# Tuee22/SpectralMC

Hardware: AMD Instinct MI355X
Metric: training-steps/sec (contracts*paths/s) + HBM GB/s, GBM 4096x65536 (higher is better)
Workload: dtype f32; 1 GPU; C2: 4096 contracts x 65536 paths (N=256 x M=256), T=16, 3-layer CVNN 6->32->32->256 fp32; contracts_per_gpu=4096, global_contracts=4096, network_size=256, batches_per_mc_run=256, assets=1, math=hw, parallelism=dp1

## Files before the change

### spectralmc_amd/csrc/gbm.hip

```cpp

#include <cmath>
#include <cstdlib>

#pragma clang fp contract(off)

#include "smc_internal.h"
#include "smc_sobol.h"
#include "smc_math.h"
#include "smc_rng.h"
#include "smc_device.h"

namespace smc {
namespace {

constexpr int kRowsWavesF64 = 4;
constexpr int kRowsWaves = 8;
constexpr int kThreads = 512;
constexpr int kWaves = kThreads / 64;
constexpr int kPathsPerLane = 4;
constexpr int kChunk = kThreads * kPathsPerLane;
constexpr double kLog2e = 1.4426950408889634;
constexpr size_t kMaxLds = 160 * 1024;

struct Contract {
  double X0, K, T, r, d, v;
};

struct EngineArgs {
  const double* contracts;
  int64_t B;
  int32_t T;
  int64_t P;
  int32_t N, M;
  uint64_t seed;
  const int64_t* ordinal_dev;
  int64_t ordinal0;
  int32_t scheme;
  int32_t normalize;
  int32_t store;
  int32_t simulate;
  int32_t all_rows;
  void* paths;
  double* rowsum;
  void* targets;
  int64_t pitch;
  int32_t slices;
  double* partials;
  uint32_t* arrivals;
  uint32_t* queues;
  const uint32_t* sobol;
  int32_t sobol_dim;
  const double* lower;
  const double* upper;
  double* contracts_out;
  float* cvnn_out;
  int64_t* cursor;
  int64_t sobol_index0;
  int64_t advance;
  uint32_t* done;
  int32_t res_slices;
  int32_t res_groups;
  uint32_t* res_cnt;
  double* res_xsum;
  double* res_xcol;
  uint32_t* res_queue;
  int32_t res_static_q = 3;
  uint32_t* status;
  uint32_t* launch_fail;
  uint32_t spin_limit;
  int32_t withhold;
};

constexpr int kSliceChunks = 4;



template <typename Real>
struct Vec4T;
template <>
struct Vec4T<float> {
  using type = float4;
};
template <>
struct Vec4T<double> {
  using type = double4;
};


__device__ __forceinline__ Contract load_contract(const double* c) {
  return Contract{c[0], c[1], c[2], c[3], c[4], c[5]};
}

__device__ __forceinline__ double wave_sum(double x) {
#pragma unroll
  for (int off = 32; off >= 1; off >>= 1) x += __shfl_xor(x, off, 64);
  return x;
}

template <typename Real, bool LOG_EULER, bool HW>
struct Stepper {
  Real a, b;

  static constexpr double zscale() {
    return sizeof(Real) == 4 && HW ? PathStream::kNormalScale<true> : 1.0;
  }

  __device__ Stepper(const Contract& c, int T) {
    const double dt = c.T / static_cast<double>(T);
    const double sq = sqrt(dt);
    if (LOG_EULER) {
      const double drift = c.r - c.d - 0.5 * c.v * c.v;
      const double scale = sizeof(Real) == 4 ? kLog2e : math::kExpUnit;
      a = static_cast<Real>(drift * dt * scale);
      b = static_cast<Real>(c.v * sq * scale * zscale());
    } else {
      a = static_cast<Real>((c.r - c.d) * dt);
      b = static_cast<Real>(c.v * sq * zscale());
    }
  }

  __device__ __forceinline__ Real operator()(Real x, Real z) const {
    if constexpr (LOG_EULER) {
      if constexpr (sizeof(Real) == 4 && HW) return x * __builtin_amdgcn_exp2f(fmaf(b, z, a));
      else if constexpr (sizeof(Real) == 4) return x * math::exp2_any(fmaf(b, z, a));
      else return math::mul_exp2s_f64(x, fma(b, z, a));
    }
    if constexpr (sizeof(Real) == 4) return fabsf(fmaf(x, fmaf(b, z, a), x));
    else return fabs(fma(x, fma(b, z, a), x));
  }
};

constexpr int kRowBlock = 16;

template <typename Real>
__device__ __forceinline__ void advance_packed(Real (&x)[4], const Real (&y)[4]) {
  typedef float f2 __attribute__((ext_vector_type(2)));
#pragma unroll
  for (int j = 0; j < 4; j += 2) {
    const f2 e = {__builtin_amdgcn_exp2f(y[j]), __builtin_amdgcn_exp2f(y[j + 1])};
    const f2 v = f2{x[j], x[j + 1]} * e;
    x[j] = v.x;
    x[j + 1] = v.y;
  }
}

template <typename Real, bool LOG_EULER, bool HW, bool ALLROWS, bool MASKED, bool FULLBLOCK, bool STRAIGHT = false,
          bool STRAIGHT_ALL = true>
__device__ __forceinline__ void lane_paths(const EngineArgs& a, const Stepper<Real, LOG_EULER, HW>& step, Real x0,
                                           uint64_t ordinal, int64_t chunk, int nvalid, int t0, int nrows,
                                           Real* contract_base, double (&acc)[ALLROWS ? kRowBlock : 1],
                                           Real* x_out = nullptr, int lid = -1) {
  using V4 = typename Vec4T<Real>::type;
  const int T = a.T;
  const int64_t P = a.P;
  const int64_t pitch = a.pitch ? a.pitch : P;
  const bool store_all = STRAIGHT ? STRAIGHT_ALL : a.store == SMC_STORE_ALL;
  const int lane_id = lid < 0 ? static_cast<int>(threadIdx.x) : lid;
  const int64_t p0 = chunk + kPathsPerLane * static_cast<int64_t>(lane_id);
  PathStream s(a.seed, ordinal, static_cast<uint64_t>(p0 / kPathsPerLane), T);
  constexpr bool kPacked = HW && LOG_EULER && sizeof(Real) == 4;
  constexpr bool kY64 = LOG_EULER && sizeof(Real) == 8;
  Real x[kPathsPerLane], zl[kPathsPerLane], zh[kPathsPerLane];
#pragma unroll
  for (int j = 0; j < kPathsPerLane; ++j) x[j] = x0;
  for (int t = 0; t < (STRAIGHT ? 0 : t0); t += 2) {
    if constexpr (kPacked) {
      s.hw_log_increments4(step.b, step.a, zl, zh);
      advance_packed(x, zl);
      advance_packed(x, zh);
    } else if constexpr (kY64) {
      s.f64_log_increments4(step.b, step.a, zl, zh);
#pragma unroll
      for (int j = 0; j < kPathsPerLane; ++j) x[j] = math::mul_exp2s_f64(math::mul_exp2s_f64(x[j], zl[j]), zh[j]);
    } else {
#pragma unroll
      for (int j = 0; j < kPathsPerLane; ++j) s.template normal_pair<HW>(zl[j], zh[j]);
#pragma unroll
      for (int j = 0; j < kPathsPerLane; ++j) x[j] = step(step(x[j], zl[j]), zh[j]);
    }
  }
  const uint32_t lane_off = static_cast<uint32_t>(kPathsPerLane * sizeof(Real)) * static_cast<uint32_t>(lane_id);
  Real* chunk_base = contract_base + chunk;
  const __amdgpu_buffer_rsrc_t contract_rsrc = row_rsrc(contract_base);
#pragma unroll
  for (int i = 0; i < kRowBlock; ++i) {
    if (FULLBLOCK || i < nrows) {
      const int t = STRAIGHT ? i : t0 + i;
      const bool tail = !FULLBLOCK && t + 1 == T;
// ... 144 lines not shown
    advance(zh);
    hook(x, t + 1);
    if constexpr (STORE_ALL) store();
    row += rstride;
  }
  if (T & 1) {
    if constexpr (kPacked) s.hw_log_tail4(step.b, step.a, zl);
    else if constexpr (kY64) s.f64_log_tail4(step.b, step.a, zl);
    else s.template normal_tail<HW>(zl);
    advance(zl);
    hook(x, T - 1);
    if constexpr (STORE_ALL) store();
  }
  if constexpr (!STORE_ALL && STORE) store();
  Real part = 0;
#pragma unroll
  for (int j = 0; j < kPathsPerLane; ++j) {
    part += x[j];
    x_out[j] = x[j];
  }
  acc += static_cast<double>(part);
}

template <typename Real, bool LOG_EULER, bool HW, bool ALLROWS>
__device__ void simulate_contract(const EngineArgs& a, const Contract& c, uint64_t ordinal, int64_t b,
                                  int64_t p_begin, int64_t p_end, double* lds_acc, double* lds_tot) {
  const int tid = threadIdx.x, lane = tid & 63, wave = tid >> 6;
  const int T = a.T;
  const int64_t P = a.P;
  const bool store_all = a.store == SMC_STORE_ALL;
  const int64_t pitch = a.pitch ? a.pitch : P;
  Real* base = static_cast<Real*>(a.paths) + (store_all ? b * T * pitch : b * pitch);
  const bool vec_ok = (P % kPathsPerLane) == 0;
  const int64_t full_end = vec_ok ? p_begin + ((p_end - p_begin) / kChunk) * kChunk : p_begin;
  const Stepper<Real, LOG_EULER, HW> step(c, T);
  const Real x0 = static_cast<Real>(c.X0);
  constexpr int kAcc = ALLROWS ? kRowBlock : 1;

  for (int t0 = 0; t0 < T; t0 += kRowBlock) {
    const int nrows = T - t0 < kRowBlock ? T - t0 : kRowBlock;
    double acc[kAcc];
#pragma unroll
    for (int i = 0; i < kAcc; ++i) acc[i] = 0.0;
    int64_t chunk = p_begin;
    if (nrows == kRowBlock) {
      if (T == kRowBlock && store_all) {
        for (; chunk < full_end; chunk += kChunk)
          lane_paths<Real, LOG_EULER, HW, ALLROWS, false, true, true>(a, step, x0, ordinal, chunk, kPathsPerLane, 0,
                                                                      kRowBlock, base, acc);
      }
      for (; chunk < full_end; chunk += kChunk)
        lane_paths<Real, LOG_EULER, HW, ALLROWS, false, true>(a, step, x0, ordinal, chunk, kPathsPerLane, t0, nrows,
                                                              base, acc);
    }
    for (; chunk < p_end; chunk += kChunk) {
      const int64_t p0 = chunk + kPathsPerLane * tid;
      const int nvalid = static_cast<int>(p0 >= p_end ? 0 : (p_end - p0 >= kPathsPerLane ? kPathsPerLane : p_end - p0));
      lane_paths<Real, LOG_EULER, HW, ALLROWS, true, false>(a, step, x0, ordinal, chunk, nvalid, t0, nrows, base,
                                                            acc);
    }
    if (ALLROWS || t0 + nrows == T) {
#pragma unroll
      for (int i = 0; i < kAcc; ++i) {
        if (i < nrows) {
          const double w = wave_sum(acc[i]);
          if (lane == 0) lds_acc[wave * kRowBlock + i] = w;
        }
      }
      __syncthreads();
      const int first = ALLROWS ? 0 : nrows - 1;
      if (tid >= first && tid < nrows) {
        double tot = 0.0;
        for (int w = 0; w < kWaves; ++w) tot += lds_acc[w * kRowBlock + (ALLROWS ? tid : 0)];
        lds_tot[t0 + tid] = tot;
      }
      __syncthreads();
    }
  }
}

template <typename Real>
struct PayoffPre {
  Real F, df, K;
  __device__ explicit PayoffPre(const Contract& c) {
    const Real Tm = static_cast<Real>(c.T);
    if constexpr (sizeof(Real) == 4) {
      F = static_cast<float>(c.X0) * math::exp_any(static_cast<float>(c.r - c.d) * Tm);
      df = math::exp_any(static_cast<float>(-c.r) * Tm);
    } else {
      F = c.X0 * exp((c.r - c.d) * Tm);
      df = exp(-c.r * Tm);
    }
    K = static_cast<Real>(c.K);
  }
};

template <typename Real>
struct Payoff {
  Real s, K, df;
  Payoff() = default;
  __device__ Payoff(const EngineArgs& a, const Contract& c, double terminal_sum)
      : Payoff(a, PayoffPre<Real>(c), terminal_sum) {}
  __device__ Payoff(const EngineArgs& a, const PayoffPre<Real>& pre, double terminal_sum) {
    df = pre.df;
    s = a.normalize ? pre.F / static_cast<Real>(terminal_sum / static_cast<double>(a.P)) : Real(1);
    K = pre.K;
    if (terminal_sum != terminal_sum) df = static_cast<Real>(__builtin_nan(""));
  }
  __device__ __forceinline__ Real operator()(Real x) const {
    const Real xs = x * s;
    const Real diff = K - xs;
    return df * (diff > Real(0) ? diff : Real(0));
  }
};

template <typename Real>
__device__ void dft_row(const double* avg, const double* cs, const double* sn, int N,
                        typename Complex2<Real>::type* out, int tid = threadIdx.x, int nthreads = kThreads) {
  using C2 = typename Complex2<Real>::type;
  const int kmax = N / 2;
  const bool fuse_nyq = (N % 2) == 0 && kmax > 0 && kmax % nthreads == 0;
  for (int k = tid; k < kmax || (!fuse_nyq && k == kmax); k += nthreads) {
    const bool nyq = fuse_nyq && k == 0;
    double re = 0.0, im = 0.0, rq = 0.0, iq = 0.0;
    int idx = 0, iqx = 0;
    for (int n = 0; n < N; ++n) {
      re = fma(avg[n], cs[idx], re);
      im = fma(-avg[n], sn[idx], im);
      idx += k;
      if (idx >= N) idx -= N;
      if (nyq) {
        rq = fma(avg[n], cs[iqx], rq);
        iq = fma(-avg[n], sn[iqx], iq);
        iqx += kmax;
        if (iqx >= N) iqx -= N;
      }
    }
    C2 v;
    v.x = static_cast<Real>(re);
    v.y = static_cast<Real>(im);
    out[k] = v;
    if (k != 0 && 2 * k != N) {
      v.y = static_cast<Real>(-im);
      out[N - k] = v;
    }
    if (nyq) {
      v.x = static_cast<Real>(rq);
      v.y = static_cast<Real>(iq);
      out[kmax] = v;
    }
  }
}

template <int kBatch>
__device__ __forceinline__ void quad_column_sums(const float* row, const Payoff<float>& pay, int N, int M,
                                                 int cols, int G, double* part, int tid, int nthreads) {
  typedef float v4f __attribute__((ext_vector_type(4)));
  const __amdgpu_buffer_rsrc_t rsrc =
      __builtin_amdgcn_make_buffer_rsrc(const_cast<float*>(row), static_cast<short>(0), 0x7fffffff, 0x00020000);
  const int items = cols * G;
  for (int item = tid; item < items; item += nthreads) {
    const int q = item % cols, g = item / cols;
    double sum[4] = {0.0, 0.0, 0.0, 0.0};
    for (int m0 = g; m0 < M; m0 += G * kBatch) {
      v4f v[kBatch];
#pragma unroll
// ... 251 lines not shown
#pragma unroll
    for (int j = 0; j < kPathsPerLane; ++j) {
      s.template normal_pair<HWN>(zl[j], zh[j]);
      if constexpr (HWN) {
        zl[j] *= kz;
        zh[j] *= kz;
      }
    }
    advance(zl);
    if constexpr (STORE_ALL) store();
    row += rstride;
    advance(zh);
    if constexpr (STORE_ALL) store();
    row += rstride;
  }
  if (T & 1) {
    s.template normal_tail<HWN>(zl);
    if constexpr (HWN) {
#pragma unroll
      for (int j = 0; j < kPathsPerLane; ++j) zl[j] *= kz;
    }
    advance(zl);
    if constexpr (STORE_ALL) store();
  }
  if constexpr (!STORE_ALL) store();
  float part = 0.0f;
#pragma unroll
  for (int j = 0; j < kPathsPerLane; ++j) part += j < nvalid ? static_cast<float>(x[j]) : 0.0f;
  acc += static_cast<double>(part);
}

constexpr int kRowsRefWaves = 6;
template <bool LOG_EULER, bool STORE_ALL, bool HWN>
__global__ __launch_bounds__(kThreads) __attribute__((amdgpu_waves_per_eu(kRowsRefWaves)))
void rows_ref_kernel(EngineArgs a) {
  extern __shared__ double lds[];
  math::f64_tables_load();
  const int64_t ord0 = (a.ordinal_dev ? *a.ordinal_dev : 0) + a.ordinal0;
  const int64_t pitch = a.pitch ? a.pitch : a.P;
  const int T = a.T;
  int parity = 0;
  for (int64_t b = blockIdx.x; b < a.B; b += gridDim.x, parity ^= 1) {
    const Contract c = load_contract(a.contracts + b * 6);
    const Stepper<double, LOG_EULER, false> step(c, T);
    float* base = static_cast<float*>(a.paths) + (STORE_ALL ? b * T * pitch : b * pitch);
    double acc = 0.0;
    for (int64_t chunk = 0; chunk < a.P; chunk += kChunk)
      lane_rows_ref<LOG_EULER, STORE_ALL, HWN>(a, step, c.X0, static_cast<uint64_t>(ord0 + b), chunk, base, T, pitch, acc);
    const double w = wave_sum(acc);
    double* ws = lds + parity * kWaves;
    if ((threadIdx.x & 63) == 0) ws[threadIdx.x >> 6] = w;
    lds_barrier();
    if (threadIdx.x == 0) {
      double tot = 0.0;
      for (int k = 0; k < kWaves; ++k) tot += ws[k];
      *pad_sum<float>(a, b) = tot;
    }
  }
}

__device__ __forceinline__ double group_sum(const double* part, int n, int G, int N) {
  double t = 0.0;
  for (int g0 = 0; g0 < G; g0 += 8) {
    double v[8];
#pragma unroll
    for (int u = 0; u < 8; ++u) v[u] = part[(g0 + u < G ? g0 + u : G - 1) * N + n];
#pragma unroll
    for (int u = 0; u < 8; ++u)
      if (g0 + u < G) t += v[u];
  }
  return t;
}

constexpr int kResThreads = 1024;
constexpr int kResWaves = kResThreads / 64;
constexpr int kResChunk = kResThreads * kPathsPerLane;
constexpr int kResMaxChunks = 16;
constexpr int kResLdsChunks = 8;
constexpr int kResRegChunks = kResMaxChunks - kResLdsChunks;
constexpr size_t kResTermBytes = static_cast<size_t>(kResLdsChunks) * kResThreads * 16;
constexpr int kResMaxSlices = 8;

constexpr int kResPreDraw = 32;
constexpr int kResMaxT = 1 << 16;

size_t resident_lds_bytes(int N) {
  return kResTermBytes +
         (static_cast<size_t>(kResWaves) + 3 * static_cast<size_t>(N) + 9 + 6 * kResPreDraw) * sizeof(double);
}

__device__ __forceinline__ void column_sums_tree(const double* part, double* red, double* avg, int N, int M) {
  const int tid = threadIdx.x, lane = tid & 63, wave = tid >> 6;
  const int R = kResThreads / N;
  const int n = tid % N, k = tid / N;
  double p = 0.0;
  if (tid < N * R) {
#pragma unroll
    for (int u = 0; u < 4; ++u) p += part[(k + u * R) * N + n];
  }
  for (int off = 32; off >= N; off >>= 1) p += __shfl_xor(p, off, 64);
  lds_barrier();
  if (N < 64) {
    if (lane < N) red[wave * N + n] = p;
  } else if (tid < N * R) {
    red[k * N + n] = p;
  }
  lds_barrier();
  const int terms = N < 64 ? kResWaves : R;
  for (int c = tid; c < N; c += kResThreads) {
    double t = 0.0;
    for (int w = 0; w < terms; ++w) t += red[w * N + c];
    avg[c] = t / static_cast<double>(M);
  }
}

template <bool LOG_EULER, bool HW, bool STORE_ALL, bool T16, bool ONTHEFLY = false>
__global__ __launch_bounds__(kResThreads) void resident_kernel(EngineArgs a) {
  static_assert(!(ONTHEFLY && T16), "the on-the-fly CF phase is instantiated for the rolled row loop only");
  typedef float v4f __attribute__((ext_vector_type(4)));
  extern __shared__ double lds[];
  const int tid = threadIdx.x, lane = tid & 63, wave = tid >> 6;
  const int N = a.N, M = a.M;
  const int64_t P = a.P;
  const int64_t pitch = a.pitch ? a.pitch : P;
  const int W = a.res_slices > 1 ? a.res_slices : 1;
  int grp = blockIdx.x, slc = 0;
  if (W > 1) {
    if (gridDim.x % (8 * W) == 0) {
      slc = static_cast<int>((blockIdx.x >> 3) % W);
      grp = static_cast<int>((blockIdx.x & 7) + 8 * (blockIdx.x / (8 * W)));
    } else {
      slc = static_cast<int>(blockIdx.x % W);
      grp = static_cast<int>(blockIdx.x / W);
    }
  }
  const int groups = static_cast<int>(gridDim.x) / W;
  const int nch = static_cast<int>(P / (static_cast<int64_t>(W) * kResChunk));
  const int cols = N / 4;
  const int G = kResChunk / N;
  const int q = tid % cols, g = tid / cols;
  v4f* term_lds = reinterpret_cast<v4f*>(lds);
  double* part = lds;
  double* wsum = lds + kResTermBytes / sizeof(double);
  double* avg = wsum + kResWaves;
  double* cs = avg + N;
  double* sn = cs + N;
  double* row = sn + N;
  double* pre = row + 9;
  for (int j = tid; j < N; j += kResThreads) math::twiddle(j, N, sn[j], cs[j]);
  const int64_t ord0 = (a.ordinal_dev ? *a.ordinal_dev : 0) + a.ordinal0;
  const int64_t sob0 = a.sobol ? a.cursor[0] + a.sobol_index0 : 0;
  uint32_t round = 0;
  const int64_t n_static0 = (a.B / groups) * a.res_static_q / 4 * groups;
  const bool dyn = a.res_queue != nullptr && (W == 1 || n_static0 > 0);
  const int64_t n_static = dyn ? n_static0 : a.B;
  auto grab = [&]() -> int64_t {
    if (tid == 0) reinterpret_cast<int64_t*>(row + 8)[0] = n_static + atomicAdd(a.res_queue, 1u);
    lds_barrier();
    return reinterpret_cast<const int64_t*>(row + 8)[0];
  };
  auto next = [&](int64_t b) -> int64_t {
    if (b + groups < n_static) return b + groups;
    if (!dyn) return a.B;
    if (W == 1) return grab();
    return reinterpret_cast<const int64_t*>(row + 8)[0];
  };
  int64_t n_pre = 0;
  if (a.sobol) {
    const int64_t mine = grp < n_static ? (n_static - 1 - grp) / groups + 1 : 0;
    n_pre = mine < kResPreDraw ? mine : kResPreDraw;
    for (int t = tid; t < n_pre * 6; t += kResThreads) {
      const int k = t / 6, d = t % 6;
      const int64_t bb = grp + static_cast<int64_t>(k) * groups;
      const double v = sobol_coord(a.sobol, a.sobol_dim, d, static_cast<uint64_t>(sob0 + bb), a.lower, a.upper);
      pre[t] = v;
      if (slc == 0) {
        a.contracts_out[bb * 6 + d] = v;
        if (a.cvnn_out) a.cvnn_out[bb * 6 + d] = static_cast<float>(v);
      }
    }
    lds_barrier();
  }
  for (int64_t b = grp < n_static ? grp : (dyn ? grab() : a.B); b < a.B; b = next(b), ++round) {
    Contract c;
    if (a.sobol && static_cast<int64_t>(round) < n_pre) {
      const double* r = pre + static_cast<int64_t>(round) * 6;
      c = Contract{r[0], r[1], r[2], r[3], r[4], r[5]};
    } else if (a.sobol) {
      if (tid < 6) {
        const double v = sobol_coord(a.sobol, a.sobol_dim, tid, static_cast<uint64_t>(sob0 + b), a.lower, a.upper);
        row[tid] = v;
        if (slc == 0) {
          a.contracts_out[b * 6 + tid] = v;
          if (a.cvnn_out) a.cvnn_out[b * 6 + tid] = static_cast<float>(v);
        }
      }
      lds_barrier();
      c = Contract{row[0], row[1], row[2], row[3], row[4], row[5]};
    } else {
      c = load_contract(a.contracts + b * 6);
    }
    const int T = T16 ? kRowBlock : a.T;
    const Stepper<float, LOG_EULER, HW> step(c, T);
    const float x0 = static_cast<float>(c.X0);
    float* base = static_cast<float*>(a.paths) + (STORE_ALL ? b * T * pitch : b * pitch);
    const int64_t p0 = static_cast<int64_t>(slc) * nch * kResChunk;
    float term[kResRegChunks][kPathsPerLane];
    double acc[1] = {0.0};
    double colsum[kPathsPerLane] = {0.0, 0.0, 0.0, 0.0};
    const PayoffPre<float> pre(c);
    const Payoff<float> pay_raw(a, pre, 1.0);
    for (int ch = 0; ch < nch; ++ch) {
      float xt[kPathsPerLane];
      if constexpr (T16)
        lane_paths<float, LOG_EULER, HW, false, false, true, true, STORE_ALL>(
            a, step, x0, static_cast<uint64_t>(ord0 + b), p0 + static_cast<int64_t>(ch) * kResChunk, kPathsPerLane,
            0, kRowBlock, base, acc, xt);
      else
        lane_rows<float, LOG_EULER, HW, STORE_ALL>(a, step, x0, static_cast<uint64_t>(ord0 + b),
                                            p0 + static_cast<int64_t>(ch) * kResChunk, base, T, pitch, acc[0], xt);
      if constexpr (ONTHEFLY) {
#pragma unroll
        for (int j = 0; j < kPathsPerLane; ++j) colsum[j] += static_cast<double>(pay_raw(xt[j]));
      } else if (ch < kResLdsChunks) {
        term_lds[ch * kResThreads + tid] = v4f{xt[0], xt[1], xt[2], xt[3]};
      } else {
#pragma unroll
        for (int i = 0; i + 1 < kResRegChunks; ++i)
#pragma unroll
          for (int j = 0; j < kPathsPerLane; ++j) term[i][j] = term[i + 1][j];
#pragma unroll
        for (int j = 0; j < kPathsPerLane; ++j) term[kResRegChunks - 1][j] = xt[j];
      }
    }
    const double w = wave_sum(acc[0]);
    if (lane == 0) wsum[wave] = w;
    lds_barrier();
    double tot = 0.0;
    {
      double wv[kResWaves];
#pragma unroll
      for (int k = 0; k < kResWaves; ++k) wv[k] = wsum[k];
#pragma unroll
      for (int k = 0; k < kResWaves; ++k) tot += wv[k];
    }
    const int64_t xslot = (static_cast<int64_t>(grp) * 2 + (round & 1)) * (W + 1);
    if (W > 1) {
      if (tid == 0) {
        put_sc1(a.res_xsum + xslot + slc, tot);
        if (dyn && slc == 0 && b + groups >= n_static)
          put_sc1(reinterpret_cast<int64_t*>(a.res_xsum + xslot + W), n_static + atomicAdd(a.res_queue, 1u));
        asm volatile("s_waitcnt vmcnt(0)" ::: "memory");
        uint32_t* cnt = a.res_cnt + static_cast<int64_t>(grp) * 64;
        if (!(a.withhold && grp == 0 && slc == W - 1 && round == 0))
          __hip_atomic_fetch_add(cnt, 1u, __ATOMIC_RELAXED, __HIP_MEMORY_SCOPE_AGENT);
        const uint32_t want = static_cast<uint32_t>(W) * (round + 1);
        uint32_t spins = 0;
        bool ok;
        while (!(ok = get_sc1(cnt) >= want) && get_sc1(a.launch_fail) == 0u && ++spins < a.spin_limit)
          __builtin_amdgcn_s_sleep(2);
        if (!ok) {
          __hip_atomic_fetch_or(a.status, SMC_SYNC_EXCHANGE_TIMEOUT, __ATOMIC_RELAXED, __HIP_MEMORY_SCOPE_AGENT);
          __hip_atomic_store(a.launch_fail, 1u, __ATOMIC_RELAXED, __HIP_MEMORY_SCOPE_AGENT);
        }
        const double t = ordered_sum_wt(a.res_xsum + xslot, 0, W, 1);
        row[6] = ok ? t : __builtin_nan("");
        if (dyn && b + groups >= n_static)
          reinterpret_cast<int64_t*>(row + 8)[0] =
              ok ? get_sc1(reinterpret_cast<const int64_t*>(a.res_xsum + xslot + W)) : a.B;
      }
      lds_barrier();
      tot = row[6];
    }
    const Payoff<float> pay(a, pre, tot);
    if constexpr (!ONTHEFLY) {
#pragma unroll
      for (int j = 0; j < kPathsPerLane; ++j) colsum[j] = 0.0;
      v4f v[kResLdsChunks];
#pragma unroll
      for (int ch = 0; ch < kResLdsChunks; ++ch) v[ch] = term_lds[ch * kResThreads + tid];
#pragma unroll
      for (int ch = 0; ch < kResLdsChunks; ++ch) {
        if (ch < nch) {
#pragma unroll
          for (int j = 0; j < kPathsPerLane; ++j) colsum[j] += static_cast<double>(pay(v[ch][j]));
        }
      }
    }
#pragma unroll
    for (int i = 0; i < kResRegChunks && !ONTHEFLY; ++i) {
      if (i >= kResRegChunks - (nch - kResLdsChunks)) {
#pragma unroll
        for (int j = 0; j < kPathsPerLane; ++j) colsum[j] += static_cast<double>(pay(term[i][j]));
      }
    }
    lds_barrier();
#pragma unroll
    for (int j = 0; j < kPathsPerLane; ++j) part[g * N + 4 * q + j] = colsum[j];
    lds_barrier();
    if (W == 1) {
      column_sums_tree(part, part, avg, N, M);
    } else {
      for (int n = tid; n < N; n += kResThreads) {
        const double t = group_sum(part, n, G, N);
        avg[n] = t;
      }
      lds_barrier();
      double* xcol = a.res_xcol + xslot * N;
      if (wave == 0) {
        for (int n = lane; n < N; n += 64) put_sc1(xcol + static_cast<int64_t>(slc) * N + n, avg[n]);
        asm volatile("s_waitcnt vmcnt(0)" ::: "memory");
        if (lane == 0) {
          const uint32_t before = __hip_atomic_fetch_add(a.res_cnt + static_cast<int64_t>(grp) * 64 + 32, 1u,
                                                         __ATOMIC_RELAXED, __HIP_MEMORY_SCOPE_AGENT);
          reinterpret_cast<int*>(row + 7)[0] = before == static_cast<uint32_t>(W) * (round + 1) - 1;
        }
      }
      lds_barrier();
      if (!reinterpret_cast<const int*>(row + 7)[0]) continue;
      for (int n = tid; n < N; n += kResThreads) avg[n] = ordered_sum_wt(xcol, n, W, N) / static_cast<double>(M);
    }
    lds_barrier();
    fft_row<float, kResThreads, true>(avg, cs, sn, N, part, part + N, static_cast<float2*>(a.targets) + b * N);
    lds_barrier();
  }
  if (a.done && tid == 0) {
    __threadfence();
    if (atomicAdd(a.done, 1u) == gridDim.x - 1) {
      a.cursor[0] += a.advance;
      a.cursor[1] += a.advance;
      if (a.res_queue) *a.res_queue = 0u;
      if (W > 1) {
        for (int k = 0; k < groups; ++k) {
          a.res_cnt[static_cast<int64_t>(k) * 64] = 0u;
          a.res_cnt[static_cast<int64_t>(k) * 64 + 32] = 0u;
        }
        *a.launch_fail = 0u;
      }
      *a.done = 0u;
    }
  }
}

constexpr int kPackMinP = 256, kPackMaxP = 2048;

size_t packed_lds_bytes(int64_t P, int N) {
  const int64_t K = kResChunk / P;
  const int64_t part = K * P > 2 * K * N ? K * P : 2 * K * N;
  return static_cast<size_t>(part + K * N + 2 * N + kResWaves + 7 * K) * sizeof(double);
}

template <bool LOG_EULER, bool HW, bool STORE_ALL, bool T16>
__global__ __launch_bounds__(kResThreads) void packed_kernel(EngineArgs a) {
  extern __shared__ double lds[];
  const int tid = threadIdx.x, lane = tid & 63, wave = tid >> 6;
  const int N = a.N, M = a.M;
  const int64_t P = a.P;
  const int64_t pitch = a.pitch ? a.pitch : P;
  const int lpc = static_cast<int>(P / kPathsPerLane);
  const int K = kResThreads / lpc;
  const int wpc = lpc / 64;
  const int k = tid / lpc, l = tid - k * lpc;
  const int cols = N / 4;
  const int q = l % cols, g = l / cols;
  const int64_t partn = K * P > 2 * K * N ? K * P : 2 * static_cast<int64_t>(K) * N;
  double* part = lds;
  double* avg = part + partn;
  double* cs = avg + K * N;
  double* sn = cs + N;
  double* wsum = sn + N;
  double* rows = wsum + kResWaves;
  for (int j = tid; j < N; j += kResThreads) math::twiddle(j, N, sn[j], cs[j]);
  const int64_t ord0 = (a.ordinal_dev ? *a.ordinal_dev : 0) + a.ordinal0;
  const int64_t sob0 = a.sobol ? a.cursor[0] + a.sobol_index0 : 0;
  const int64_t ngroups = (a.B + K - 1) / K;
  for (int64_t grp = blockIdx.x; grp < ngroups; grp += gridDim.x) {
    const int64_t b0 = grp * K;
    const int kv = a.B - b0 < K ? static_cast<int>(a.B - b0) : K;
    if (tid < 6 * kv) {
      const int kk = tid / 6, d = tid - 6 * kk;
      double v;
      if (a.sobol) {
        v = sobol_coord(a.sobol, a.sobol_dim, d, static_cast<uint64_t>(sob0 + b0 + kk), a.lower, a.upper);
        a.contracts_out[(b0 + kk) * 6 + d] = v;
        if (a.cvnn_out) a.cvnn_out[(b0 + kk) * 6 + d] = static_cast<float>(v);
      } else {
        v = a.contracts[(b0 + kk) * 6 + d];
      }
      rows[kk * 7 + d] = v;
    }
    lds_barrier();
    const bool active = k < kv;
    const double* r = rows + (active ? k : 0) * 7;
    const Contract c{r[0], r[1], r[2], r[3], r[4], r[5]};
    const int T = T16 ? kRowBlock : a.T;
    float xt[kPathsPerLane] = {0.0f, 0.0f, 0.0f, 0.0f};
    double acc[1] = {0.0};
    if (active) {
      const Stepper<float, LOG_EULER, HW> step(c, T);
      const float x0 = static_cast<float>(c.X0);
      const int64_t b = b0 + k;
      float* base = static_cast<float*>(a.paths) + (STORE_ALL ? b * T * pitch : b * pitch);
      if constexpr (T16)
        lane_paths<float, LOG_EULER, HW, false, false, true, true, STORE_ALL>(
            a, step, x0, static_cast<uint64_t>(ord0 + b), 0, kPathsPerLane, 0, kRowBlock, base, acc, xt, l);
      else
        lane_rows<float, LOG_EULER, HW, STORE_ALL>(a, step, x0, static_cast<uint64_t>(ord0 + b), 0, base, T, pitch,
                                                   acc[0], xt, l);
    }
    const double w = wave_sum(acc[0]);
    if (lane == 0) wsum[wave] = w;
    lds_barrier();
    if (tid < K) {
      double tot = 0.0;
      for (int v = 0; v < wpc; ++v) tot += wsum[tid * wpc + v];
// ... 868 lines not shown

size_t workspace_bytes(int64_t B, int32_t T, int64_t P, bool all_rows) {
  const int64_t W = slices_for(P, true);
  if (W <= 1) return 0;
  return static_cast<size_t>(B) * W * (all_rows ? T : 1) * sizeof(double) + static_cast<size_t>(B + 16) * sizeof(uint32_t);
}

constexpr int kPathsWgsPerCu = 4;

template <bool LOG_EULER, bool HW, bool STRAIGHT, bool STORE_ALL>
int32_t launch_split_k(const EngineArgs& a, hipStream_t stream) {
  const size_t lds1 = lds_bytes(a.T, a.N, false), lds2 = lds_bytes(a.T, a.N, true);
  auto k1 = paths_kernel<LOG_EULER, HW, STRAIGHT, STORE_ALL>;
  auto k2 = cf_kernel<float>;
  if ((lds1 > 64 * 1024 && hipFuncSetAttribute(reinterpret_cast<const void*>(k1),
                                                hipFuncAttributeMaxDynamicSharedMemorySize,
                                                static_cast<int>(lds1)) != hipSuccess) ||
      (lds2 > 64 * 1024 && hipFuncSetAttribute(reinterpret_cast<const void*>(k2),
                                                hipFuncAttributeMaxDynamicSharedMemorySize,
                                                static_cast<int>(lds2)) != hipSuccess)) {
    (void)hipGetLastError();
    return fail(SMC_ERR_HIP, "paths_kernel / cf_kernel: cannot raise the dynamic LDS limit");
  }
  unsigned grid1 = static_cast<unsigned>(a.B);
  if (STRAIGHT) {
    int dev = 0, cus = 0;
    if (hipGetDevice(&dev) != hipSuccess ||
        hipDeviceGetAttribute(&cus, hipDeviceAttributeMultiprocessorCount, dev) != hipSuccess || cus <= 0) {
      (void)hipGetLastError();
      return fail(SMC_ERR_HIP, "paths_kernel: device query failed");
    }
    const int64_t slots = static_cast<int64_t>(kPathsWgsPerCu) * cus;
    if (slots < a.B) grid1 = static_cast<unsigned>(slots);
  }
  launch(k1, dim3(grid1), dim3(kThreads), lds1, stream, a);
  if (int32_t st = check_launch("paths_kernel")) return st;
  launch(k2, dim3(static_cast<unsigned>(a.B)), dim3(kThreads), lds2, stream, a);
  return check_launch("cf_kernel");
}

template <typename Real, bool LOG_EULER, bool HW, bool STORE_ALL>
int32_t launch_rows_k(const EngineArgs& a, hipStream_t stream) {
  const size_t lds1 = 2 * kWaves * sizeof(double), lds2 = lds_bytes(a.T, a.N, true);
  auto k1 = rows_kernel<Real, LOG_EULER, HW, STORE_ALL>;
  auto k2 = cf_kernel<Real>;
  if (lds2 > kMaxLds) return fail(SMC_ERR_INVALID_SHAPE, "engine: network_size exceeds the LDS budget");
  if (lds2 > 64 * 1024 && hipFuncSetAttribute(reinterpret_cast<const void*>(k2),
                                               hipFuncAttributeMaxDynamicSharedMemorySize,
                                               static_cast<int>(lds2)) != hipSuccess) {
    (void)hipGetLastError();
    return fail(SMC_ERR_HIP, "cf_kernel: cannot raise the dynamic LDS limit");
  }
  unsigned grid1 = 0;
  if (int32_t st = resident_grid(reinterpret_cast<const void*>(k1), kThreads, lds1, a.B, &grid1)) return st;
  launch(k1, dim3(grid1), dim3(kThreads), lds1, stream, a);
  if (int32_t st = check_launch("rows_kernel")) return st;
  launch(k2, dim3(static_cast<unsigned>(a.B)), dim3(kThreads), lds2, stream, a);
  return check_launch("cf_kernel");
}

template <bool LOG_EULER, bool STORE_ALL, bool HWN>
int32_t launch_rows_ref_k(const EngineArgs& a, hipStream_t stream) {
  const size_t lds1 = 2 * kWaves * sizeof(double), lds2 = lds_bytes(a.T, a.N, true);
  auto k1 = rows_ref_kernel<LOG_EULER, STORE_ALL, HWN>;
  auto k2 = cf_kernel<float>;
  if (lds2 > kMaxLds) return fail(SMC_ERR_INVALID_SHAPE, "engine: network_size exceeds the LDS budget");
  if (lds2 > 64 * 1024 && hipFuncSetAttribute(reinterpret_cast<const void*>(k2),
                                               hipFuncAttributeMaxDynamicSharedMemorySize,
                                               static_cast<int>(lds2)) != hipSuccess) {
    (void)hipGetLastError();
    return fail(SMC_ERR_HIP, "cf_kernel: cannot raise the dynamic LDS limit");
  }
  unsigned grid1 = 0;
  if (int32_t st = resident_grid(reinterpret_cast<const void*>(k1), kThreads, lds1, a.B, &grid1)) return st;
  launch(k1, dim3(grid1), dim3(kThreads), lds1, stream, a);
  if (int32_t st = check_launch("rows_ref_kernel")) return st;
  launch(k2, dim3(static_cast<unsigned>(a.B)), dim3(kThreads), lds2, stream, a);
  return check_launch("cf_kernel");
}

template <bool LOG_EULER, bool HW, bool STORE_ALL>
int32_t launch_resident_k(const EngineArgs& a, hipStream_t stream) {
  const int W = a.res_slices > 1 ? a.res_slices : 1;
  auto kernel = a.T == kRowBlock                 ? resident_kernel<LOG_EULER, HW, STORE_ALL, true>
                : (!a.normalize && W == 1) ? resident_kernel<LOG_EULER, HW, STORE_ALL, false, true>
                                           : resident_kernel<LOG_EULER, HW, STORE_ALL, false>;
  const size_t lds = resident_lds_bytes(a.N);
  if (lds > 64 * 1024 && hipFuncSetAttribute(reinterpret_cast<const void*>(kernel),
                                             hipFuncAttributeMaxDynamicSharedMemorySize,
                                             static_cast<int>(lds)) != hipSuccess) {
    (void)hipGetLastError();
    return fail(SMC_ERR_HIP, "resident_kernel: cannot raise the dynamic LDS limit");
  }
  unsigned grid = 0;
  if (int32_t st = resident_grid(reinterpret_cast<const void*>(kernel), kResThreads, lds, a.B * W, &grid, stream))
    return st;
  if (W > 1) {
    unsigned groups = grid / W;
    if (groups > static_cast<unsigned>(a.res_groups)) groups = static_cast<unsigned>(a.res_groups);
    if (groups >= 8) groups -= groups % 8;
    if (groups == 0) return fail(SMC_ERR_INVALID_SHAPE, "resident_kernel: fewer resident slots than slices");
    grid = groups * W;
  }
  launch(kernel, dim3(grid), dim3(kResThreads), lds, stream, a);
  return check_launch("resident_kernel");
}

template <bool LOG_EULER, bool HW, bool STORE_ALL>
int32_t launch_wave_k(const EngineArgs& a, hipStream_t stream) {
  auto kernel = a.T == 1 ? wave_kernel<LOG_EULER, HW, STORE_ALL, 1> : wave_kernel<LOG_EULER, HW, STORE_ALL, 2>;
  const size_t lds = wave_lds_bytes(a.N);
  if (lds > 64 * 1024 && hipFuncSetAttribute(reinterpret_cast<const void*>(kernel),
                                             hipFuncAttributeMaxDynamicSharedMemorySize,
                                             static_cast<int>(lds)) != hipSuccess) {
    (void)hipGetLastError();
    return fail(SMC_ERR_HIP, "wave_kernel: cannot raise the dynamic LDS limit");
  }
  unsigned grid = 0;
  const int64_t wpg = kWaveThreads / 64;
  if (int32_t st = resident_grid(reinterpret_cast<const void*>(kernel), kWaveThreads, lds, (a.B + wpg - 1) / wpg, &grid,
                                 stream))
    return st;
  launch(kernel, dim3(grid), dim3(kWaveThreads), lds, stream, a);
  return check_launch("wave_kernel");
}

template <bool LOG_EULER, bool HW, bool STORE_ALL>
int32_t launch_packed_k(const EngineArgs& a, hipStream_t stream) {
  auto kernel = a.T == kRowBlock ? packed_kernel<LOG_EULER, HW, STORE_ALL, true>
                                 : packed_kernel<LOG_EULER, HW, STORE_ALL, false>;
  const size_t lds = packed_lds_bytes(a.P, a.N);
  if (lds > kMaxLds) return fail(SMC_ERR_INVALID_SHAPE, "packed_kernel: network_size exceeds the LDS budget");
  if (lds > 64 * 1024 && hipFuncSetAttribute(reinterpret_cast<const void*>(kernel),
                                             hipFuncAttributeMaxDynamicSharedMemorySize,
                                             static_cast<int>(lds)) != hipSuccess) {
    (void)hipGetLastError();
    return fail(SMC_ERR_HIP, "packed_kernel: cannot raise the dynamic LDS limit");
  }
  const int64_t K = kResChunk / a.P;
  unsigned grid = 0;
  if (int32_t st = resident_grid(reinterpret_cast<const void*>(kernel), kResThreads, lds, (a.B + K - 1) / K, &grid,
                                 stream))
    return st;
  launch(kernel, dim3(grid), dim3(kResThreads), lds, stream, a);
  return check_launch("packed_kernel");
}


template <typename Real>
int32_t launch_engine(EngineArgs a, hipStream_t stream) {
  if (a.B == 0) return SMC_OK;
  if ((a.scheme & SMC_MATH_REF) != 0) {
    if (sizeof(Real) != 4) return fail(SMC_ERR_INVALID_ARGUMENT, "engine: SMC_MATH_REF is an f32 mode");
    if (!ref_ok(a))
      return fail(SMC_ERR_INVALID_SHAPE, "engine: SMC_MATH_REF needs targets, whole contracts per workgroup and "
                                         "a padded pitch (smc_path_pitch)");
    const bool log_euler = (a.scheme & 0xff) == SMC_SCHEME_LOG_EULER;
    const bool sa = a.store == SMC_STORE_ALL;
    if ((a.scheme & SMC_MATH_HW) != 0) {
      if (log_euler)
        return sa ? launch_rows_ref_k<true, true, true>(a, stream) : launch_rows_ref_k<true, false, true>(a, stream);
      return sa ? launch_rows_ref_k<false, true, true>(a, stream) : launch_rows_ref_k<false, false, true>(a, stream);
    }
    if (log_euler)
      return sa ? launch_rows_ref_k<true, true, false>(a, stream) : launch_rows_ref_k<true, false, false>(a, stream);
    return sa ? launch_rows_ref_k<false, true, false>(a, stream) : launch_rows_ref_k<false, false, false>(a, stream);
  }
  if constexpr (sizeof(Real) == 4) {
    if (wave_ok(a, true)) {
// ... 712 lines not shown
```

Baseline: 99.97 billion contracts*paths/s.

## Overlap next-contract prep and single-wave FFT in resident kernel, split sliced variant

Adds a SLICED template parameter so the unsliced resident kernel compiles without the cross-slice branches. In the unsliced path, one dedicated wave computes the next contract's stepper and payoff constants (Sobol draw, queue ticket) into LDS while wave 0 performs the column mean and FFT for N<=256. This hides per-contract setup and removes several block-wide barriers. It also uses ds_bpermute for wave reductions and simplifies the column-sum indexing. The risks are serialising the FFT onto a single wave and added complexity in the queue/ticket handoff.

New measurement: 101.3 billion contracts*paths/s (median of 5 runs). Within noise of the previous version (+1.3%).

```diff
diff --git a/spectralmc_amd/csrc/gbm.hip b/spectralmc_amd/csrc/gbm.hip
--- a/spectralmc_amd/csrc/gbm.hip
+++ b/spectralmc_amd/csrc/gbm.hip
@@ -97,6 +97,20 @@
   return x;
 }
 
+__device__ __forceinline__ double lane_xor(double x, int lane, int off) {
+  const int addr = ((lane & 63) ^ off) << 2;
+  const uint64_t u = __builtin_bit_cast(uint64_t, x);
+  const uint32_t lo = static_cast<uint32_t>(__builtin_amdgcn_ds_bpermute(addr, static_cast<int>(u)));
+  const uint32_t hi = static_cast<uint32_t>(__builtin_amdgcn_ds_bpermute(addr, static_cast<int>(u >> 32)));
+  return __builtin_bit_cast(double, static_cast<uint64_t>(hi) << 32 | lo);
+}
+
+__device__ __forceinline__ double wave_sum(double x, int lane) {
+#pragma unroll
+  for (int off = 32; off >= 1; off >>= 1) x += lane_xor(x, lane, off);
+  return x;
+}
+
 template <typename Real, bool LOG_EULER, bool HW>
 struct Stepper {
   Real a, b;
@@ -104,6 +118,8 @@
   static constexpr double zscale() {
     return sizeof(Real) == 4 && HW ? PathStream::kNormalScale<true> : 1.0;
   }
+
+  __device__ Stepper(Real a_, Real b_) : a(a_), b(b_) {}
 
   __device__ Stepper(const Contract& c, int T) {
     const double dt = c.T / static_cast<double>(T);
@@ -414,6 +430,7 @@
 template <typename Real>
 struct PayoffPre {
   Real F, df, K;
+  __device__ PayoffPre(Real F_, Real df_, Real K_) : F(F_), df(df_), K(K_) {}
   __device__ explicit PayoffPre(const Contract& c) {
     const Real Tm = static_cast<Real>(c.T);
     if constexpr (sizeof(Real) == 4) {
@@ -831,6 +848,7 @@
 constexpr int kResMaxSlices = 8;
 
 constexpr int kResPreDraw = 32;
+constexpr int kResWaveFft = 256;
 constexpr int kResMaxT = 1 << 16;
 
 size_t resident_lds_bytes(int N) {
@@ -838,43 +856,45 @@
          (static_cast<size_t>(kResWaves) + 3 * static_cast<size_t>(N) + 9 + 6 * kResPreDraw) * sizeof(double);
 }
 
-__device__ __forceinline__ void column_sums_tree(const double* part, double* red, double* avg, int N, int M) {
-  const int tid = threadIdx.x, lane = tid & 63, wave = tid >> 6;
+__device__ __forceinline__ void column_sums_tree(const double* part, double* red, int N, int tid) {
+  const int lane = tid & 63, wave = tid >> 6;
   const int R = kResThreads / N;
-  const int n = tid % N, k = tid / N;
+  const int n = tid & (N - 1), k = tid / N;
   double p = 0.0;
   if (tid < N * R) {
 #pragma unroll
     for (int u = 0; u < 4; ++u) p += part[(k + u * R) * N + n];
   }
-  for (int off = 32; off >= N; off >>= 1) p += __shfl_xor(p, off, 64);
-  lds_barrier();
+  for (int off = 32; off >= N; off >>= 1) p += lane_xor(p, lane, off);
   if (N < 64) {
     if (lane < N) red[wave * N + n] = p;
   } else if (tid < N * R) {
     red[k * N + n] = p;
   }
-  lds_barrier();
-  const int terms = N < 64 ? kResWaves : R;
-  for (int c = tid; c < N; c += kResThreads) {
+}
+
+__device__ __forceinline__ void column_sums_mean(const double* red, double* avg, int N, int M, int tid, int nthreads) {
+  const int terms = N < 64 ? kResWaves : kResThreads / N;
+  for (int c = tid; c < N; c += nthreads) {
     double t = 0.0;
     for (int w = 0; w < terms; ++w) t += red[w * N + c];
     avg[c] = t / static_cast<double>(M);
   }
 }
 
-template <bool LOG_EULER, bool HW, bool STORE_ALL, bool T16, bool ONTHEFLY = false>
+template <bool LOG_EULER, bool HW, bool STORE_ALL, bool T16, bool ONTHEFLY = false, bool SLICED = false>
 __global__ __launch_bounds__(kResThreads) void resident_kernel(EngineArgs a) {
   static_assert(!(ONTHEFLY && T16), "the on-the-fly CF phase is instantiated for the rolled row loop only");
+  static_assert(!(ONTHEFLY && SLICED), "the on-the-fly CF phase is for whole contracts");
   typedef float v4f __attribute__((ext_vector_type(4)));
   extern __shared__ double lds[];
-  const int tid = threadIdx.x, lane = tid & 63, wave = tid >> 6;
+  const int tid = threadIdx.x, lane = tid & 63, wave = __builtin_amdgcn_readfirstlane(tid >> 6);
   const int N = a.N, M = a.M;
   const int64_t P = a.P;
   const int64_t pitch = a.pitch ? a.pitch : P;
-  const int W = a.res_slices > 1 ? a.res_slices : 1;
+  const int W = SLICED ? a.res_slices : 1;
   int grp = blockIdx.x, slc = 0;
-  if (W > 1) {
+  if constexpr (SLICED) {
     if (gridDim.x % (8 * W) == 0) {
       slc = static_cast<int>((blockIdx.x >> 3) % W);
       grp = static_cast<int>((blockIdx.x & 7) + 8 * (blockIdx.x / (8 * W)));
@@ -885,9 +905,7 @@
   }
   const int groups = static_cast<int>(gridDim.x) / W;
   const int nch = static_cast<int>(P / (static_cast<int64_t>(W) * kResChunk));
-  const int cols = N / 4;
   const int G = kResChunk / N;
-  const int q = tid % cols, g = tid / cols;
   v4f* term_lds = reinterpret_cast<v4f*>(lds);
   double* part = lds;
   double* wsum = lds + kResTermBytes / sizeof(double);
@@ -896,12 +914,18 @@
   double* sn = cs + N;
   double* row = sn + N;
   double* pre = row + 9;
+  constexpr int kPrepWave = kResWaves - 1;
+  float* kc = reinterpret_cast<float*>(row);
+  const int T = T16 ? kRowBlock : a.T;
+  auto uniform = [](float x) {
+    return __builtin_bit_cast(float, __builtin_amdgcn_readfirstlane(__builtin_bit_cast(int, x)));
+  };
   for (int j = tid; j < N; j += kResThreads) math::twiddle(j, N, sn[j], cs[j]);
   const int64_t ord0 = (a.ordinal_dev ? *a.ordinal_dev : 0) + a.ordinal0;
   const int64_t sob0 = a.sobol ? a.cursor[0] + a.sobol_index0 : 0;
   uint32_t round = 0;
   const int64_t n_static0 = (a.B / groups) * a.res_static_q / 4 * groups;
-  const bool dyn = a.res_queue != nullptr && (W == 1 || n_static0 > 0);
+  const bool dyn = a.res_queue != nullptr && (!SLICED || n_static0 > 0);
   const int64_t n_static = dyn ? n_static0 : a.B;
   auto grab = [&]() -> int64_t {
     if (tid == 0) reinterpret_cast<int64_t*>(row + 8)[0] = n_static + atomicAdd(a.res_queue, 1u);
@@ -911,7 +935,6 @@
   auto next = [&](int64_t b) -> int64_t {
     if (b + groups < n_static) return b + groups;
     if (!dyn) return a.B;
-    if (W == 1) return grab();
     return reinterpret_cast<const int64_t*>(row + 8)[0];
   };
   int64_t n_pre = 0;
@@ -930,35 +953,81 @@
     }
     lds_barrier();
   }
-  for (int64_t b = grp < n_static ? grp : (dyn ? grab() : a.B); b < a.B; b = next(b), ++round) {
+  auto prepare = [&](int64_t nb, int64_t r) {
+    int d = lane;
+    asm volatile("" : "+v"(d));
     Contract c;
-    if (a.sobol && static_cast<int64_t>(round) < n_pre) {
-      const double* r = pre + static_cast<int64_t>(round) * 6;
-      c = Contract{r[0], r[1], r[2], r[3], r[4], r[5]};
+    if (a.sobol && r < n_pre) {
+      const double* p = pre + r * 6;
+      c = Contract{p[0], p[1], p[2], p[3], p[4], p[5]};
     } else if (a.sobol) {
-      if (tid < 6) {
-        const double v = sobol_coord(a.sobol, a.sobol_dim, tid, static_cast<uint64_t>(sob0 + b), a.lower, a.upper);
-        row[tid] = v;
-        if (slc == 0) {
-          a.contracts_out[b * 6 + tid] = v;
-          if (a.cvnn_out) a.cvnn_out[b * 6 + tid] = static_cast<float>(v);
+      double v = 0.0;
+      if (d < 6) {
+        v = sobol_coord(a.sobol, a.sobol_dim, d, static_cast<uint64_t>(sob0 + nb), a.lower, a.upper);
+        a.contracts_out[nb * 6 + d] = v;
+        if (a.cvnn_out) a.cvnn_out[nb * 6 + d] = static_cast<float>(v);
+      }
+      c = Contract{__shfl(v, 0, 64), __shfl(v, 1, 64), __shfl(v, 2, 64),
+                   __shfl(v, 3, 64), __shfl(v, 4, 64), __shfl(v, 5, 64)};
+    } else {
+      c = load_contract(a.contracts + nb * 6);
+    }
+    const Stepper<float, LOG_EULER, HW> st(c, T);
+    const PayoffPre<float> pp(c);
+    if (d == 0) {
+      kc[0] = st.a;
+      kc[1] = st.b;
+      kc[2] = static_cast<float>(c.X0);
+      kc[3] = pp.F;
+      kc[4] = pp.df;
+      kc[5] = pp.K;
+    }
+  };
+  int64_t b = grp < n_static ? grp : (dyn ? grab() : a.B);
+  if constexpr (!SLICED) {
+    if (wave == kPrepWave && b < a.B) prepare(b, 0);
+    lds_barrier();
+  }
+  uint32_t ticket;
+  asm volatile("" : "=v"(ticket));
+  for (; b < a.B; b = next(b), ++round) {
+    float sa, sb, x0, pF, pdf, pK;
+    if constexpr (!SLICED) {
+      sa = kc[0], sb = kc[1], x0 = kc[2], pF = kc[3], pdf = kc[4], pK = kc[5];
+    } else {
+      Contract c;
+      if (a.sobol && static_cast<int64_t>(round) < n_pre) {
+        const double* r = pre + static_cast<int64_t>(round) * 6;
+        c = Contract{r[0], r[1], r[2], r[3], r[4], r[5]};
+      } else if (a.sobol) {
+        int d = tid;
+        asm volatile("" : "+v"(d));
+        if (d < 6) {
+          const double v = sobol_coord(a.sobol, a.sobol_dim, d, static_cast<uint64_t>(sob0 + b), a.lower, a.upper);
+          row[d] = v;
+          if (slc == 0) {
+            a.contracts_out[b * 6 + d] = v;
+            if (a.cvnn_out) a.cvnn_out[b * 6 + d] = static_cast<float>(v);
+          }
         }
-      }
-      lds_barrier();
-      c = Contract{row[0], row[1], row[2], row[3], row[4], row[5]};
-    } else {
-      c = load_contract(a.contracts + b * 6);
-    }
-    const int T = T16 ? kRowBlock : a.T;
-    const Stepper<float, LOG_EULER, HW> step(c, T);
-    const float x0 = static_cast<float>(c.X0);
+        lds_barrier();
+        c = Contract{row[0], row[1], row[2], row[3], row[4], row[5]};
+      } else {
+        c = load_contract(a.contracts + b * 6);
+      }
+      const Stepper<float, LOG_EULER, HW> st(c, T);
+      const PayoffPre<float> pp(c);
+      sa = st.a, sb = st.b, x0 = static_cast<float>(c.X0), pF = pp.F, pdf = pp.df, pK = pp.K;
+    }
+    const Stepper<float, LOG_EULER, HW> step(uniform(sa), uniform(sb));
+    x0 = uniform(x0);
+    const PayoffPre<float> ppre(uniform(pF), uniform(pdf), uniform(pK));
     float* base = static_cast<float*>(a.paths) + (STORE_ALL ? b * T * pitch : b * pitch);
     const int64_t p0 = static_cast<int64_t>(slc) * nch * kResChunk;
     float term[kResRegChunks][kPathsPerLane];
     double acc[1] = {0.0};
     double colsum[kPathsPerLane] = {0.0, 0.0, 0.0, 0.0};
-    const PayoffPre<float> pre(c);
-    const Payoff<float> pay_raw(a, pre, 1.0);
+    const Payoff<float> pay_raw(a, ppre, 1.0);
     for (int ch = 0; ch < nch; ++ch) {
       float xt[kPathsPerLane];
       if constexpr (T16)
@@ -982,8 +1051,16 @@
         for (int j = 0; j < kPathsPerLane; ++j) term[kResRegChunks - 1][j] = xt[j];
       }
     }
-    const double w = wave_sum(acc[0]);
-    if (lane == 0) wsum[wave] = w;
+    int ct = tid;
+    asm volatile("" : "+v"(ct));
+    const double w = wave_sum(acc[0], ct);
+    if ((ct & 63) == 0) wsum[wave] = w;
+    const bool tail = dyn && b + groups >= n_static;
+    if (!SLICED && tail && wave == kPrepWave && (ct & 63) == 0) {
+      uint32_t* queue = a.res_queue;
+      asm volatile("" : "+v"(queue));
+      ticket = atomicAdd(queue, 1u);
+    }
     lds_barrier();
     double tot = 0.0;
     {
@@ -994,7 +1071,7 @@
       for (int k = 0; k < kResWaves; ++k) tot += wv[k];
     }
     const int64_t xslot = (static_cast<int64_t>(grp) * 2 + (round & 1)) * (W + 1);
-    if (W > 1) {
+    if constexpr (SLICED) {
       if (tid == 0) {
         put_sc1(a.res_xsum + xslot + slc, tot);
         if (dyn && slc == 0 && b + groups >= n_static)
@@ -1021,13 +1098,13 @@
       lds_barrier();
       tot = row[6];
     }
-    const Payoff<float> pay(a, pre, tot);
+    const Payoff<float> pay(a, ppre, tot);
     if constexpr (!ONTHEFLY) {
 #pragma unroll
       for (int j = 0; j < kPathsPerLane; ++j) colsum[j] = 0.0;
       v4f v[kResLdsChunks];
 #pragma unroll
-      for (int ch = 0; ch < kResLdsChunks; ++ch) v[ch] = term_lds[ch * kResThreads + tid];
+      for (int ch = 0; ch < kResLdsChunks; ++ch) v[ch] = term_lds[ch * kResThreads + ct];
 #pragma unroll
       for (int ch = 0; ch < kResLdsChunks; ++ch) {
         if (ch < nch) {
@@ -1045,10 +1122,34 @@
     }
     lds_barrier();
 #pragma unroll
-    for (int j = 0; j < kPathsPerLane; ++j) part[g * N + 4 * q + j] = colsum[j];
+    for (int j = 0; j < kPathsPerLane; ++j) part[4 * ct + j] = colsum[j];
     lds_barrier();
-    if (W == 1) {
-      column_sums_tree(part, part, avg, N, M);
+    if constexpr (!SLICED) {
+      double* red = part + kResChunk;
+      column_sums_tree(part, red, N, ct);
+      lds_barrier();
+      __builtin_amdgcn_s_waitcnt(0x0F70);
+      if (wave == kPrepWave) {
+        const int64_t nb = b + groups < n_static
+                               ? b + groups
+                               : (tail ? n_static + static_cast<uint32_t>(__builtin_amdgcn_readfirstlane(ticket)) : a.B);
+        if (nb < a.B) prepare(nb, static_cast<int64_t>(round) + 1);
+        if ((ct & 63) == 0) reinterpret_cast<int64_t*>(row + 8)[0] = nb;
+        __builtin_amdgcn_s_waitcnt(0x0F70);
+      }
+      float2* out = static_cast<float2*>(a.targets) + b * N;
+      if (N <= kResWaveFft) {
+        if (wave == 0) {
+          column_sums_mean(red, avg, N, M, ct & 63, 64);
+          wave_lds_sync();
+          fft_rows<float, 64, true, true>(avg, cs, sn, N, 1, 1, part, part + N, out);
+        }
+      } else {
+        column_sums_mean(red, avg, N, M, ct, kResThreads);
+        lds_barrier();
+        fft_row<float, kResThreads, true>(avg, cs, sn, N, part, part + N, out);
+      }
+      lds_barrier();
     } else {
       for (int n = tid; n < N; n += kResThreads) {
         const double t = group_sum(part, n, G, N);
@@ -1068,10 +1169,10 @@
       lds_barrier();
       if (!reinterpret_cast<const int*>(row + 7)[0]) continue;
       for (int n = tid; n < N; n += kResThreads) avg[n] = ordered_sum_wt(xcol, n, W, N) / static_cast<double>(M);
-    }
-    lds_barrier();
-    fft_row<float, kResThreads, true>(avg, cs, sn, N, part, part + N, static_cast<float2*>(a.targets) + b * N);
-    lds_barrier();
+      lds_barrier();
+      fft_row<float, kResThreads, true>(avg, cs, sn, N, part, part + N, static_cast<float2*>(a.targets) + b * N);
+      lds_barrier();
+    }
   }
   if (a.done && tid == 0) {
     __threadfence();
@@ -1079,7 +1180,7 @@
       a.cursor[0] += a.advance;
       a.cursor[1] += a.advance;
       if (a.res_queue) *a.res_queue = 0u;
-      if (W > 1) {
+      if constexpr (SLICED) {
         for (int k = 0; k < groups; ++k) {
           a.res_cnt[static_cast<int64_t>(k) * 64] = 0u;
           a.res_cnt[static_cast<int64_t>(k) * 64 + 32] = 0u;
@@ -2114,9 +2215,11 @@
 template <bool LOG_EULER, bool HW, bool STORE_ALL>
 int32_t launch_resident_k(const EngineArgs& a, hipStream_t stream) {
   const int W = a.res_slices > 1 ? a.res_slices : 1;
-  auto kernel = a.T == kRowBlock                 ? resident_kernel<LOG_EULER, HW, STORE_ALL, true>
-                : (!a.normalize && W == 1) ? resident_kernel<LOG_EULER, HW, STORE_ALL, false, true>
-                                           : resident_kernel<LOG_EULER, HW, STORE_ALL, false>;
+  auto kernel = W > 1 ? (a.T == kRowBlock ? resident_kernel<LOG_EULER, HW, STORE_ALL, true, false, true>
+                                          : resident_kernel<LOG_EULER, HW, STORE_ALL, false, false, true>)
+                : a.T == kRowBlock ? resident_kernel<LOG_EULER, HW, STORE_ALL, true>
+                : !a.normalize     ? resident_kernel<LOG_EULER, HW, STORE_ALL, false, true>
+                                   : resident_kernel<LOG_EULER, HW, STORE_ALL, false>;
   const size_t lds = resident_lds_bytes(a.N);
   if (lds > 64 * 1024 && hipFuncSetAttribute(reinterpret_cast<const void*>(kernel),
                                              hipFuncAttributeMaxDynamicSharedMemorySize,
```
